# rlav440/pyCamSet

Hardware: AMD Instinct MI355X
Metric: residual+Jacobian rows/sec (higher is better)
Workload: dtype f64; 1 GPU; rig-32 (BASELINE config 3): 32 cams x 200 poses x 486 keys, 998401 detections, chain template; detections_total=998401, detections_per_gpu=998401, row_len_P=21, collective_in_step=none, parallelism=obs-shard x1

## Files before the change

pycamset_amd/csrc/ba_device.hpp:

```cpp
#pragma once
#ifndef __HIPCC_RTC__
#include <hip/hip_runtime.h>

#include <cstdint>
#else
#include "ba_rtc_prelude.hpp"
#endif

namespace pcs {

constexpr int CHAIN_TEMPLATE = 0;
constexpr int CHAIN_SELF = 1;
constexpr int CHAIN_FREE = 2;

__host__ __device__ constexpr int chain_P(int chain) { return chain == CHAIN_TEMPLATE ? 21 : chain == CHAIN_SELF ? 24 : 18; }

constexpr int CAM_STRIDE = 48;
constexpr int POSE_STRIDE = 40;
constexpr int CAM_R = 9, CAM_T = 18, CAM_DR = 21;
constexpr int POSE_R = 0, POSE_T = 9, POSE_DR = 12;

struct DetTable {
    const uint32_t *packed;
    const int32_t *cam, *img, *key;
// ... 260 lines not shown
                for (int aa = 0; aa < 3; ++aa) J[i * P + 15 + aa] = S[i][0] * Qr[0 * 3 + aa] + S[i][1] * Qr[1 * 3 + aa] + S[i][2] * Qr[2 * 3 + aa];
#pragma unroll
                for (int c = 0; c < 3; ++c) J[i * P + 18 + c] = S[i][c];
            }
            if constexpr (CHAIN == CHAIN_SELF) {
#pragma unroll
                for (int i = 0; i < 2; ++i)
#pragma unroll
                    for (int c = 0; c < 3; ++c)
                        J[i * P + 21 + c] = S[i][0] * ps[POSE_R + 0 * 3 + c] + S[i][1] * ps[POSE_R + 1 * 3 + c] + S[i][2] * ps[POSE_R + 2 * 3 + c];
            }
        }
    }
}

template <int CHAIN, typename SlabPtrC, typename SlabPtrP, typename MatPtr, typename VecPtr>
__device__ __forceinline__ void eval_detection_jvp(SlabPtrC cs, SlabPtrP ps, const double X0, const double X1, const double X2, MatPtr M, VecPtr vi,
                                                   VecPtr vet, VecPtr vpt, const double vX0, const double vX1, const double vX2, double &du, double &dv) {
    double Xw0, Xw1, Xw2, dW0, dW1, dW2;
    if constexpr (CHAIN != CHAIN_FREE) {
        const double r0 = ps[POSE_R + 0], r1 = ps[POSE_R + 1], r2 = ps[POSE_R + 2];
        const double r3 = ps[POSE_R + 3], r4 = ps[POSE_R + 4], r5 = ps[POSE_R + 5];
        const double r6 = ps[POSE_R + 6], r7 = ps[POSE_R + 7], r8 = ps[POSE_R + 8];
        Xw0 = r0 * X0 + r1 * X1 + r2 * X2 + ps[POSE_T + 0];
        Xw1 = r3 * X0 + r4 * X1 + r5 * X2 + ps[POSE_T + 1];
        Xw2 = r6 * X0 + r7 * X1 + r8 * X2 + ps[POSE_T + 2];
        dW0 = M[9] * X0 + M[10] * X1 + M[11] * X2 + vpt[0];
        dW1 = M[12] * X0 + M[13] * X1 + M[14] * X2 + vpt[1];
        dW2 = M[15] * X0 + M[16] * X1 + M[17] * X2 + vpt[2];
        if constexpr (CHAIN == CHAIN_SELF) {
// ... 38 lines not shown
```

pycamset_amd/csrc/ba_normal.hpp:

```cpp
#pragma once
#include <hip/hip_runtime.h>

#include <cstddef>

#include "ba_device.hpp"
#include "ba_matfree.hpp"

namespace pcs {

struct NormalArgs {
    DetTable tab;
    const int32_t *order;
    const void *cam_slab, *pose_slab, *points;
    double *H;
    double *HB, *HC;
    double *g;
    double *cost;
    int32_t ldA, ldB, tb;
    int32_t trail_group;
    int64_t trail_off;
    int64_t n, n_tiles;
    int64_t extr_off, pose_off, point_off;
    int64_t n_params;
    int32_t tiles_per_wave;
    const int32_t *stop;
    const int32_t *sel;
    int64_t alt;
    double *part;
    const int32_t *seg_base;
    int32_t loss;
    double inv_f_scale, f_scale_sq;
    double *wave_cost;
    int32_t debug;
    const double *inv_sigma;
};

constexpr int PASS_SHARED = 0, PASS_CAMKEY = 1, PASS_IMGKEY = 2;
constexpr int NORMAL_R = 30;
constexpr int normal_shared_cols(int chain) { return chain == CHAIN_FREE ? 15 : 21; }
constexpr int normal_slots(int chain, int pass) {
    return pass == PASS_SHARED ? normal_shared_cols(chain) + 1 : pass == PASS_CAMKEY ? 19 : 9;
}
constexpr int normal_mfmas(int chain, int pass) { return (pass == PASS_SHARED && chain != CHAIN_FREE) ? 2 : 1; }
constexpr int normal_slot_stride(int rows) { return 2 * rows * 8 + 8; }
constexpr int normal_lds_bytes(int chain, int pass, int rows) { return normal_slots(chain, pass) * normal_slot_stride(rows) + 128; }

template <int CHAIN, int PASS>
__host__ __device__ __forceinline__ constexpr int slot_col(int s) {
    constexpr int NS = normal_shared_cols(CHAIN);
    if (PASS == PASS_SHARED) return s < NS ? s : NORMAL_R;
    if (PASS == PASS_CAMKEY) return s < 15 ? s : s < 18 ? NS + (s - 15) : NORMAL_R;
    return s < 6 ? 15 + s : NS + (s - 6);
}

template <int CHAIN, int PASS>
__host__ __device__ __forceinline__ int window_slot(int w, int j) {
    if (PASS == PASS_SHARED) {
        if (CHAIN == CHAIN_FREE) return j;
        if (w == 1) return j;
        const int g = w == 0 ? 0 : 8;
        return j < 8 ? g + j : j < 14 ? 16 + (j - 8) : -1;
    }
    if (PASS == PASS_CAMKEY) {
        if (w == 0) return j < 3 ? 15 + j : j == 3 ? 18 : j - 4;
        return j < 3 ? 15 + j : j < 6 ? 12 + (j - 3) : -1;
    }
    if (w == 0) return j < 6 ? j : -1;
    return j < 3 ? 6 + j : -1;
}
template <int CHAIN, int PASS> constexpr int n_windows() { return (PASS == PASS_SHARED) ? (CHAIN == CHAIN_FREE ? 1 : 3) : 2; }
template <int CHAIN, int PASS> __host__ __device__ __forceinline__ constexpr int mfma_a(int m) { return PASS == PASS_SHARED ? (CHAIN == CHAIN_FREE ? 0 : m == 0 ? 0 : 2) : 0; }
template <int CHAIN, int PASS> __host__ __device__ __forceinline__ constexpr int mfma_b(int m) { return PASS == PASS_SHARED ? (CHAIN == CHAIN_FREE ? 0 : m == 0 ? 1 : 2) : 1; }

template <int CHAIN, int PASS>
__host__ __device__ __forceinline__ bool entry_kept(int m, int i, int j, int &sa, int &sb) {
    sa = window_slot<CHAIN, PASS>(mfma_a<CHAIN, PASS>(m), i);
    sb = window_slot<CHAIN, PASS>(mfma_b<CHAIN, PASS>(m), j);
    if (sa < 0 || sb < 0) return false;
    if (PASS == PASS_SHARED) {
        if (CHAIN == CHAIN_FREE) return i <= j;
        if (m == 0) return i >= 8 || i <= j;
        return i <= j && !(i < 8 && j >= 8);
    }
    if (PASS == PASS_CAMKEY) {
        if (i < 3) return j >= 3 || i <= j;
        return j < 3;
    }
    return true;
}

template <int CHAIN, int PASS>
__host__ __device__ __forceinline__ int entry_descriptor(const int m, const int lane, const int r, const int tg) {
    constexpr bool HAS_POSE = CHAIN != CHAIN_FREE;
    constexpr int NS = normal_shared_cols(CHAIN);
    auto col_group = [](const int lc) -> int { return lc == NORMAL_R ? 4 : lc < 9 ? 0 : lc < 15 ? 1 : (HAS_POSE && lc < NS) ? 2 : 3; };
    auto col_offset = [](const int lc) -> int { return lc == NORMAL_R ? 0 : lc < 9 ? lc : lc < 15 ? lc - 9 : (HAS_POSE && lc < NS) ? lc - 15 : lc - NS; };
    int sa, sb;
    const bool keep = entry_kept<CHAIN, PASS>(m, (lane >> 4) + 4 * r, lane & 15, sa, sb);
    const int la = slot_col<CHAIN, PASS>(keep ? sa : 0), lb = slot_col<CHAIN, PASS>(keep ? sb : 0);
    int gR = col_group(la), oR = col_offset(la), gC = col_group(lb), oC = col_offset(lb);
    const bool pose = PASS == PASS_SHARED && (gR == 2 || gC == 2);
    if (gR > gC || (gR == gC && oR > oC)) { int t = gR; gR = gC; gC = t; t = oR; oR = oC; oC = t; }
    int eRow, eCol, eLd, ePtr;
    if (gR == 4) { oR = 0; oC = 0; eRow = 9; eCol = 9; eLd = 15; ePtr = 4; }
    else if (gC == 4) { oC = oR; oR = 0; eRow = 9; eCol = 24 + gR; eLd = 15; ePtr = 3; }
    else if (gR == tg) { eRow = 8; eCol = 9; eLd = 14; ePtr = 2; }
    else if (gC == tg) { eRow = 4 + gR; eCol = 16 + gC; eLd = 13; ePtr = 1; }
    else { eRow = gR; eCol = 16 + gC; eLd = 12; ePtr = 0; }
    return oR | (oC << 4) | (eRow << 8) | (eCol << 13) | (eLd << 18) | (ePtr << 23) | (keep ? 1 << 27 : 0) | (pose ? 1 << 28 : 0);
}

template <int CHAIN, int PASS, int KS>
__device__ __attribute__((noinline)) double2v robust_scale_row(const int kind, const double r0, const double r1, const double inv_f_scale,
                                                               const double f_scale_sq, const double *inv_sigma_tab, const int idx, unsigned char *dst) {
    const double inv_sigma = inv_sigma_tab ? inv_sigma_tab[idx] : 1.0;
    double q0, q1, f0, f1;
    const double s0 = robust_rho<true>(kind, r0 * inv_sigma, inv_f_scale, f_scale_sq, q0, f0) * inv_sigma;
    const double s1 = robust_rho<true>(kind, r1 * inv_sigma, inv_f_scale, f_scale_sq, q1, f1) * inv_sigma;
#pragma unroll
    for (int s = 0; s < normal_slots(CHAIN, PASS); ++s) {
        double *q = reinterpret_cast<double *>(dst + s * KS);
        if (slot_col<CHAIN, PASS>(s) == NORMAL_R) {
            q[0] = f0;
            q[1] = f1;
        } else {
            q[0] *= s0;
            q[1] *= s1;
        }
    }
    return double2v{q0, q1};
}

using d4v = __attribute__((ext_vector_type(4))) double;

template <int CHAIN, int PASS, int ROWS>
__global__ __launch_bounds__(64, 2) void ba_normal_mfma_kernel(const NormalArgs a) {
    static_assert(ROWS == 64 || ROWS == 32, "image holds a whole or half a tile");
    static_assert(PASS == PASS_SHARED || CHAIN != CHAIN_TEMPLATE, "the template chain has no point columns");
    static_assert(PASS != PASS_IMGKEY || CHAIN == CHAIN_SELF, "only the self chain couples poses and points");
    using T = double;
    constexpr int P = chain_P(CHAIN);
    constexpr int P2 = 2 * P;
    constexpr int NSLOT = normal_slots(CHAIN, PASS);
    constexpr int NW = n_windows<CHAIN, PASS>();
    constexpr int NM = normal_mfmas(CHAIN, PASS);
    constexpr int KS = normal_slot_stride(ROWS);
    constexpr int STEPS = ROWS / 2;
    constexpr bool HAS_POSE = CHAIN != CHAIN_FREE;
    using D2 = __attribute__((ext_vector_type(2))) double;

    extern __shared__ __attribute__((aligned(16))) unsigned char lds_image[];
    if (a.stop && *a.stop) return;
    const int lane = threadIdx.x;
    const T *cam_slab = static_cast<const T *>(a.cam_slab);
    const T *pose_slab = static_cast<const T *>(a.pose_slab);
    const T *points = static_cast<const T *>(a.points);

    int rd_off[NW];
#pragma unroll
    for (int w = 0; w < NW; ++w) {
        const int s = window_slot<CHAIN, PASS>(w, lane & 15);
        rd_off[w] = (s < 0 ? 0 : s) * KS + (lane >> 4) * 8;
    }
    const int tg = a.trail_group;
    int ent[NM][4];
#pragma unroll
    for (int m = 0; m < NM; ++m)
#pragma unroll
        for (int r = 0; r < 4; ++r) ent[m][r] = entry_descriptor<CHAIN, PASS>(m, lane, r, tg);
    const bool robust = a.loss != LOSS_LINEAR;
    if (PASS == PASS_SHARED && robust) {
#pragma unroll
        for (int m = 0; m < NM; ++m)
#pragma unroll
            for (int r = 0; r < 4; ++r)
                if (((ent[m][r] >> 23) & 7) == 4) ent[m][r] &= ~(1 << 27);
    }
    double rho_acc = 0.0;
    const int64_t out_shift = (a.sel && *a.sel) ? 8 * a.alt : 0;
    const uint64_t out_ptr = (lane == 1 ? (uint64_t)a.HB : lane == 2 ? (uint64_t)a.HC : lane == 3 ? (uint64_t)a.g : lane == 4 ? (uint64_t)a.cost : (uint64_t)a.H) + (uint64_t)out_shift;
    const int ptr_lo = (int)(uint32_t)out_ptr, ptr_hi = (int)(uint32_t)(out_ptr >> 32);
    int base_tab = lane == 12 ? a.ldA : lane == 13 ? a.ldB : lane == 14 ? a.tb : 0;
    d4v acc[NM];
#pragma unroll
    for (int m = 0; m < NM; ++m) acc[m] = d4v{0.0, 0.0, 0.0, 0.0};

    int run_a = -1, run_b = -1;

    int64_t seg = a.part ? a.seg_base[blockIdx.x] : 0;
    auto flush = [&](const bool everything) {
        if (run_a < 0) return;
        if (a.part) {
            double *slot = a.part + seg * (NM * 256) + lane;
#pragma unroll
            for (int m = 0; m < NM; ++m)
#pragma unroll
                for (int r = 0; r < 4; ++r) {
                    slot[(m * 4 + r) * 64] = acc[m][r];
                    acc[m][r] = 0.0;
                }
            ++seg;
            return;
        }
        if (a.debug & 128) {
#pragma unroll
            for (int m = 0; m < NM; ++m)
#pragma unroll
                for (int r = 0; r < 4; ++r) acc[m][r] = (everything || (ent[m][r] & (1 << 28))) ? 0.0 : acc[m][r];
            return;
        }
        const int cam = PASS == PASS_IMGKEY ? 0 : run_a;
        const int img = PASS == PASS_SHARED ? run_b : run_a;
        const int key = run_b;
        const int base[4] = {9 * cam, (int)a.extr_off + 6 * cam, (int)a.pose_off + 6 * img, (int)a.point_off + 3 * key};
#pragma unroll
        for (int g = 0; g < 4; ++g) {
            const uint32_t b = (uint32_t)__builtin_amdgcn_readfirstlane(base[g]);
            const int rowA = (int)((uint32_t)a.ldA * b), rowB = (int)((uint32_t)a.ldB * b);
            const int col = (int)(b - (g == tg ? (uint32_t)a.trail_off : 0u)), gi = (int)b;
            asm("v_writelane_b32 %0, %1, %2" : "+v"(base_tab) : "s"(rowA), "n"(g));
            asm("v_writelane_b32 %0, %1, %2" : "+v"(base_tab) : "s"(rowB), "n"(4 + g));
            asm("v_writelane_b32 %0, %1, %2" : "+v"(base_tab) : "s"(col), "n"(16 + g));
            asm("v_writelane_b32 %0, %1, %2" : "+v"(base_tab) : "s"(gi), "n"(24 + g));
        }
        {
            const int ent_idx = tg == 2 ? img : key;
            const int rowC = __builtin_amdgcn_readfirstlane((int)((uint32_t)(a.tb * a.tb) * (uint32_t)ent_idx));
            asm("v_writelane_b32 %0, %1, %2" : "+v"(base_tab) : "s"(rowC), "n"(8));
        }
        uint64_t dst[NM][4];
        int dsc[NM][4];
#pragma unroll
        for (int m = 0; m < NM; ++m)
#pragma unroll
            for (int r = 0; r < 4; ++r) {
                int d = ent[m][r];
                asm volatile("" : "+v"(d));
                const uint32_t ld = (uint32_t)__builtin_amdgcn_ds_bpermute((d >> 16) & (31 << 2), base_tab);
                const uint32_t off = (uint32_t)__builtin_amdgcn_ds_bpermute((d >> 6) & (31 << 2), base_tab) +
                                     (uint32_t)__builtin_amdgcn_ds_bpermute((d >> 11) & (31 << 2), base_tab) +
                                     ((uint32_t)(d & 15) * ld + (uint32_t)((d >> 4) & 15));
                const int psel = (d >> 21) & (7 << 2);
                const uint64_t pb = ((uint64_t)(uint32_t)__builtin_amdgcn_ds_bpermute(psel, ptr_hi) << 32) | (uint32_t)__builtin_amdgcn_ds_bpermute(psel, ptr_lo);
                dst[m][r] = pb + ((uint64_t)off << 3);
                dsc[m][r] = d;
            }
#pragma unroll
        for (int m = 0; m < NM; ++m)
#pragma unroll
            for (int r = 0; r < 4; ++r) {
                const int d = dsc[m][r];
                const bool now = everything || (d & (1 << 28));
                const double s = acc[m][r];
                acc[m][r] = now ? 0.0 : s;
                if (now && (d & (1 << 27)) && s != 0.0 && !(a.debug & 2))
                    __builtin_amdgcn_global_atomic_fadd_f64(reinterpret_cast<__attribute__((address_space(1))) double *>(dst[m][r]), s);
            }
    };

    const int64_t tile0 = (int64_t)blockIdx.x * a.tiles_per_wave;
    const int64_t tile1 = min(tile0 + (int64_t)a.tiles_per_wave, a.n_tiles);
    auto det_index = [&](const int64_t tile) -> int64_t {
        const int64_t i = tile * 64 + lane;
        const int64_t is = i < a.n ? i : a.n - 1;
        return a.order ? a.order[is] : is;
    };
    DetWords nxt_w{};
    double2v nxt_m{};
    if (tile0 < tile1) {
// ... 13 lines not shown
            nxt_w = load_words(a.tab, icn);
            nxt_m = load_uv(a.tab, icn);
        }
        asm volatile("" ::: "memory");
        T u, v;
        T J[P2];
        if (a.debug & 16) {
            u = m.x; v = m.y;
#pragma unroll
            for (int j = 0; j < P2; ++j) J[j] = m.x + (double)j;
        } else {
            const T X0 = points[3 * k], X1 = points[3 * k + 1], X2 = points[3 * k + 2];
            const int c0 = __builtin_amdgcn_readfirstlane(c), im0 = __builtin_amdgcn_readfirstlane(im);
            const bool cam_uni = __all(c == c0), img_uni = !HAS_POSE || __all(im == im0);
            const T *csp = cam_slab + c * CAM_STRIDE, *psp = pose_slab + im * POSE_STRIDE;
            if (PASS == PASS_SHARED && cam_uni && img_uni) {
                const LaneSlab lc{cam_slab[c0 * CAM_STRIDE + min(lane, CAM_STRIDE - 1)]};
                const LaneSlab lp{HAS_POSE ? pose_slab[im0 * POSE_STRIDE + min(lane, POSE_STRIDE - 1)] : 0.0};
                eval_detection<CHAIN, T, true>(lc, lp, X0, X1, X2, u, v, J);
            } else if (PASS == PASS_CAMKEY && cam_uni) {
                const LaneSlab lc{cam_slab[c0 * CAM_STRIDE + min(lane, CAM_STRIDE - 1)]};
                eval_detection<CHAIN, T, true>(lc, psp, X0, X1, X2, u, v, J);
            } else if (PASS == PASS_IMGKEY && img_uni) {
                const LaneSlab lp{pose_slab[im0 * POSE_STRIDE + min(lane, POSE_STRIDE - 1)]};
                eval_detection<CHAIN, T, true>(csp, lp, X0, X1, X2, u, v, J);
            } else {
                eval_detection<CHAIN, T, true>(csp, psp, X0, X1, X2, u, v, J);
            }
        }
        const double r0 = u - m.x, r1 = v - m.y;
        asm volatile("" ::"v"(nxt_w.w0), "v"(nxt_w.w1), "v"(nxt_w.w2), "v"(nxt_m.x), "v"(nxt_m.y));

        const int ka = PASS == PASS_IMGKEY ? im : c, kb = PASS == PASS_SHARED ? im : k;
        const int pa = __shfl_up(ka, 1), pb = __shfl_up(kb, 1);
        const bool starts = valid && (lane == 0 ? (ka != run_a || kb != run_b) : (ka != pa || kb != pb));
        const uint64_t bnd = __ballot(starts);

#pragma unroll
        for (int h = 0; h < 64 / ROWS; ++h) {
            if (!(a.debug & 64) && (ROWS == 64 || (lane >> 5) == h)) {
                unsigned char *dst = lds_image + (lane & (ROWS - 1)) * 16;
#pragma unroll
                for (int s = 0; s < NSLOT; ++s) {
                    const int lc = slot_col<CHAIN, PASS>(s);
                    double *q = reinterpret_cast<double *>(dst + s * KS);
                    q[0] = lc == NORMAL_R ? r0 : J[lc];
                    q[1] = lc == NORMAL_R ? r1 : J[P + lc];
                }
                if (!valid) {
#pragma unroll
                    for (int s = 0; s < NSLOT; ++s) {
                        double *q = reinterpret_cast<double *>(dst + s * KS);
                        q[0] = 0.0;
                        q[1] = 0.0;
                    }
                } else if (robust) {
                    int w_off = (int)offsetof(NormalArgs, inv_sigma);
                    asm volatile("" : "+s"(w_off));
                    using KernArg = const __attribute__((address_space(4))) char *;
                    const double *inv_sigma = *reinterpret_cast<const double *const __attribute__((address_space(4))) *>((KernArg)__builtin_amdgcn_kernarg_segment_ptr() + w_off);
                    const int det = (int)tile * 64 + lane;
                    const double2v q = robust_scale_row<CHAIN, PASS, KS>(a.loss, r0, r1, a.inv_f_scale, a.f_scale_sq, inv_sigma, a.order ? a.order[det] : det, dst);
                    if (PASS == PASS_SHARED) {
                        if (a.loss == LOSS_CAUCHY || a.loss == LOSS_ARCTAN)
                            rho_acc += a.f_scale_sq * robust_rho_transcendental(a.loss, q.x) + a.f_scale_sq * robust_rho_transcendental(a.loss, q.y);
                        else
                            rho_acc += q.x + q.y;
                    }
                }
            }
            __builtin_amdgcn_fence(__ATOMIC_RELEASE, "wavefront");
            __builtin_amdgcn_wave_barrier();
            __builtin_amdgcn_fence(__ATOMIC_ACQUIRE, "wavefront");

            const int d_base = h * ROWS;
            const uint64_t bits = (a.debug & 32) ? 0ull : ROWS == 64 ? bnd : (bnd >> d_base) & 0xffffffffull;
            auto operand = [&](const int w, const int s) { return *reinterpret_cast<const double *>(lds_image + rd_off[w] + s * 32); };
            auto run_mfmas = [&](const double (&x)[NW]) {
#pragma unroll
                for (int mm = 0; mm < NM; ++mm)
                    acc[mm] = __builtin_amdgcn_mfma_f64_16x16x4f64(x[mfma_a<CHAIN, PASS>(mm)], x[mfma_b<CHAIN, PASS>(mm)], acc[mm], 0, 0, 0);
            };
            auto new_run = [&](const int d) {
                const int na = __builtin_amdgcn_readlane(ka, d), nb = __builtin_amdgcn_readlane(kb, d);
                flush(PASS != PASS_SHARED || na != run_a);
                run_a = na;
                run_b = nb;
            };
            const uint32_t lds_base = (uint32_t)(uintptr_t)(__attribute__((address_space(3))) unsigned char *)lds_image;
            auto run_steps = [&](const int s0, const int s1) {
                if (s0 >= s1) return;
                double x[3][NW];
                using LdsD = const __attribute__((address_space(3))) double *;
                uint32_t adr[NW];
#pragma unroll
                for (int w = 0; w < NW; ++w) {
                    adr[w] = lds_base + (uint32_t)rd_off[w] + (uint32_t)s0 * 32u;
                    asm volatile("" : "+v"(adr[w]));
                    x[0][w] = *(LdsD)(uintptr_t)adr[w];
                    x[1][w] = *(LdsD)(uintptr_t)(adr[w] + 32u);
// ... 47 lines not shown
                        run_mfmas(xa);
                        new_run(d0 + 1);
                        run_mfmas(xb);
                    } else {
                        run_mfmas(x);
                    }
                    s0 = sb + 1;
                }
            }
            __builtin_amdgcn_fence(__ATOMIC_RELEASE, "wavefront");
            __builtin_amdgcn_wave_barrier();
            __builtin_amdgcn_fence(__ATOMIC_ACQUIRE, "wavefront");
        }
    }
    flush(true);
    if (PASS == PASS_SHARED && robust) {
        const double c = wave_sum(rho_acc);
        if (lane == 0) {
            if (a.part) a.wave_cost[blockIdx.x] = c;
            else if (c != 0.0 && !(a.debug & 2)) unsafeAtomicAdd(a.cost + out_shift / 8, c);
        }
    }
}

constexpr int IK_COLS = 6;
constexpr int IK_SLOT = 64 * 8 + 16;
constexpr int IK_RUNS = IK_COLS * IK_SLOT;
constexpr int IK_GRAM = IK_RUNS + 65 * 16;
constexpr int normal_imgkey_lds_bytes() { return IK_GRAM + 64 * IK_COLS * 8; }

__global__ __launch_bounds__(64, 3) void ba_normal_imgkey_kernel(const NormalArgs a) {
// ... 168 lines not shown
```

pycamset_amd/csrc/pcs_common.inc:

```

static thread_local std::string g_err;

static int fail(int code, const char *fmt, ...) {
    char buf[512];
    va_list ap;
    va_start(ap, fmt);
    vsnprintf(buf, sizeof buf, fmt, ap);
    va_end(ap);
    g_err = buf;
    return code;
}

#define HIPCHK(expr)                                                                              \
    do {                                                                                          \
        hipError_t _e = (expr);                                                                   \
        if (_e != hipSuccess) return fail(PCS_ERR_HIP, "%s failed: %s (%s:%d)", #expr, hipGetErrorString(_e), __FILE__, __LINE__); \
    } while (0)

static int device_cu_count(int device) {
    static std::atomic<int> cached[64];
    if (device < 0 || device >= 64) return 0;
    int v = cached[device].load();
    if (v == 0) {
        if (hipDeviceGetAttribute(&v, hipDeviceAttributeMultiprocessorCount, device) != hipSuccess) v = 0;
        cached[device].store(v);
    }
    return v;
}

extern "C" {
int pcs_version(void) { return 128; }
const char *pcs_last_error(void) { return g_err.c_str(); }

int pcs_device_count(void) {
    int n = 0;
    if (hipGetDeviceCount(&n) != hipSuccess) return 0;
    return n;
}

int pcs_host_alloc(void **out, int64_t bytes) {
    if (!out || bytes <= 0) return fail(PCS_ERR_ARG, "pcs_host_alloc: bad arguments");
    *out = nullptr;
    HIPCHK(hipHostMalloc(out, (size_t)bytes, hipHostMallocDefault));
    return PCS_OK;
}

// ... 50 lines not shown
```

pycamset_amd/csrc/pcs_engine.hip:

```cpp
#include <hip/hip_ext.h>
#include <hip/hip_runtime.h>

#include <atomic>

#include <algorithm>
#include <array>
#include <cmath>
#include <cstdarg>
#include <cstdint>
#include <cstdio>
#include <cstdlib>
#include <cstring>
#include <initializer_list>
#include <string>
#include <vector>

#include "../../include/pcs_hip.h"
#include "ba_device.hpp"
#include "ba_kernels.hpp"
#include "ba_matfree.hpp"
#include "ba_normal.hpp"
#include "ba_reduce.hpp"
#include "ba_schur.hpp"
#include "ba_lm_fused.hpp"
// ... 93 lines not shown
    int normal_imgkey_product = 1;
    bool matfree_lds = true;
    int n_cu = 256;
    int variant = -1;
    int64_t wgs_per_cu = 0;
    int compact_variant = 1;
    bool xcd_remap = false;
    double tile_locality = 1.0;
    double tile_segments = 1.0;
    int fuse_prep = -1;
    int64_t fuse_prep_max_n = 250000;
    int64_t tiles_per_wg = 0;
    size_t lds_limit = 160 * 1024;
    int64_t spd_timeout_us = 250000;
    int deterministic = 0;
    int loss = 0;
    double f_scale = 1.0;
    int fused_trial = 1;
    std::vector<int32_t> h_order, h_order_ck;
    struct DetPass {
        int64_t n = -1;
        int64_t tpw = 0;
        int32_t n_seg = 0, n_lr = 0, n_grp = 0, n_ent = 0, n_waves = 0;
        int32_t *d_idx = nullptr;
        int64_t off[9] = {};
        double *d_work = nullptr;
        int64_t work_off[4] = {};
    } det_pass[2];
};

// ... 281 lines not shown
        HIPCHK(hipSetDevice(h->device));
        HIPCHK(wait_done_host(h));
        for (auto &e : h->ev)
            if (e) (void)hipEventDestroy(e);
        h->ev.assign(4 * value, nullptr);
        h->ev_has_prep.assign(value, 0);
        for (auto &e : h->ev) HIPCHK(hipEventCreate(&e));
        h->ev_ring = value;
        h->ev_count = 0;
        h->events_valid = false;
    } else if (!strcmp(key, "fused_trial")) {
        h->fused_trial = value != 0;
    } else if (!strcmp(key, "deterministic")) {
        if (value < 0 || value > 1) return fail(PCS_ERR_ARG, "deterministic must be 0 or 1");
        h->deterministic = (int)value;
    } else if (!strcmp(key, "spd_timeout_us")) {
        if (value < 1 || value > 60000000) return fail(PCS_ERR_ARG, "spd_timeout_us must be in [1, 60000000]");
        h->spd_timeout_us = value;
    } else if (!strcmp(key, "tiles_per_wg")) {
        if (value < 0 || value > (1 << 20)) return fail(PCS_ERR_ARG, "tiles_per_wg out of range");
        h->tiles_per_wg = value;
    } else {
        return fail(PCS_ERR_ARG, "pcs_set_option: unknown key '%s'", key);
    }
    return PCS_OK;
}

static_assert(PCS_LOSS_LINEAR == LOSS_LINEAR && PCS_LOSS_HUBER == LOSS_HUBER && PCS_LOSS_SOFT_L1 == LOSS_SOFT_L1 && PCS_LOSS_CAUCHY == LOSS_CAUCHY &&
              PCS_LOSS_ARCTAN == LOSS_ARCTAN, "loss kinds of the C ABI and of ba_device.hpp");
int pcs_set_loss(pcs_engine *h, int kind, double f_scale) {
// ... 219 lines not shown
    switch (chain) {
        case CHAIN_TEMPLATE: return launch_matfree_c<CHAIN_TEMPLATE, false>(op, a, grid, 0, s);
        case CHAIN_SELF: return launch_matfree_c<CHAIN_SELF, false>(op, a, grid, 0, s);
        default: return launch_matfree_c<CHAIN_FREE, false>(op, a, grid, 0, s);
    }
}

template <int CHAIN, int PASS>
static hipError_t launch_normal_p(int rows, const NormalArgs &a, dim3 grid, hipStream_t s) {
    if (rows == 32) hipLaunchKernelGGL((ba_normal_mfma_kernel<CHAIN, PASS, 32>), grid, dim3(64), normal_lds_bytes(CHAIN, PASS, 32), s, a);
    else hipLaunchKernelGGL((ba_normal_mfma_kernel<CHAIN, PASS, 64>), grid, dim3(64), normal_lds_bytes(CHAIN, PASS, 64), s, a);
    return hipGetLastError();
}

static hipError_t launch_normal(int chain, int pass, int rows, const NormalArgs &a, dim3 grid, hipStream_t s) {
    if (pass == PASS_SHARED) {
        switch (chain) {
            case CHAIN_TEMPLATE: return launch_normal_p<CHAIN_TEMPLATE, PASS_SHARED>(rows, a, grid, s);
            case CHAIN_SELF: return launch_normal_p<CHAIN_SELF, PASS_SHARED>(rows, a, grid, s);
            default: return launch_normal_p<CHAIN_FREE, PASS_SHARED>(rows, a, grid, s);
        }
    }
    if (pass == PASS_CAMKEY)
        return chain == CHAIN_SELF ? launch_normal_p<CHAIN_SELF, PASS_CAMKEY>(rows, a, grid, s) : launch_normal_p<CHAIN_FREE, PASS_CAMKEY>(rows, a, grid, s);
    return launch_normal_p<CHAIN_SELF, PASS_IMGKEY>(rows, a, grid, s);
}

template <typename E>
__global__ void gather_rows_kernel(const int32_t *__restrict__ order, const E *__restrict__ src, E *__restrict__ dst, int64_t n) {
    const int64_t i = (int64_t)blockIdx.x * blockDim.x + threadIdx.x;
// ... 325 lines not shown
                const pcs_engine::DetPass &D = h->det_pass[pass];
                if ((int64_t)grid.x != D.n_waves) return fail(PCS_ERR_STATE, "deterministic mode: launch geometry and segment table disagree");
                a.part = D.d_work + D.work_off[0];
                a.seg_base = D.d_idx + D.off[0];
                a.wave_cost = D.d_work + D.work_off[3];
                e = launch_normal(h->chain, pass, h->normal_rows, a, grid, s);
                if (e == hipSuccess) {
                    ReduceArgs ra{};
                    ra.part = a.part; ra.Q = D.d_work + D.work_off[1]; ra.G = D.d_work + D.work_off[2];
                    ra.lr_ptr = D.d_idx + D.off[1]; ra.lr_segs = D.d_idx + D.off[2]; ra.lr_ka = D.d_idx + D.off[3]; ra.lr_kb = D.d_idx + D.off[4];
                    ra.grp_ptr = D.d_idx + D.off[5]; ra.cam_ptr = D.d_idx + D.off[6]; ra.ent_ptr = D.d_idx + D.off[7]; ra.ent_runs = D.d_idx + D.off[8];
                    ra.n_lr = D.n_lr; ra.n_grp = D.n_grp; ra.n_cams = (int32_t)h->n_cams; ra.n_ent = D.n_ent; ra.n_waves = D.n_waves;
                    e = launch_reduce(h->chain, pass, a, ra, s);
                }
            } else {
                e = launch_normal(h->chain, pass, h->normal_rows, a, grid, s);
            }
        }
        if (e != hipSuccess) return fail(PCS_ERR_HIP, "normal-equations kernel launch failed: %s", hipGetErrorString(e));
    }
    if (timed) {
        HIPCHK(hipEventRecord(ev[3], s));
        ++h->ev_count;
        h->events_valid = true;
    }
    HIPCHK(mark_done(h, s));
    return PCS_OK;
}

static int enqueue_eval(pcs_engine *h, const double *d_prm, void *d_resid, void *d_out, bool compact, hipStream_t s) {
    if (h->det.n <= 0) return fail(PCS_ERR_STATE, "no detections set");
// ... 594 lines not shown
```

Baseline: 32.26 billion rows/s.

## Accumulate shared-pass normal equations in a 16-column twist basis, fold back per run

Adds a twist-basis shared pass: each detection's Jacobian is formed against 15 columns (intrinsics plus a 6-dof combined-rigid twist), so the MFMA Gram product uses one 16-wide window instead of three windows and two MFMAs. Per run, a noinline fold routine maps the twist Gram back to the camera/pose parameter columns using LDS scratch and per-run rotation data, then issues atomics. It is enabled by default for non-free chains in the non-deterministic path. It trades cheaper per-row Jacobian and MFMA work for extra per-run fold cost, LDS use and atomics. The metric here is residual+Jacobian rows, so it is unclear whether the normal pass is even timed.

```diff
diff --git a/pycamset_amd/csrc/ba_device.hpp b/pycamset_amd/csrc/ba_device.hpp
--- a/pycamset_amd/csrc/ba_device.hpp
+++ b/pycamset_amd/csrc/ba_device.hpp
@@ -298,6 +298,65 @@
     }
 }
 
+constexpr int NORMAL_TWIST_COLS = 16;
+template <int CHAIN, typename SlabPtrC, typename SlabPtrP>
+__device__ __forceinline__ void eval_detection_twist(SlabPtrC cs, SlabPtrP ps, const double X0, const double X1, const double X2, double &u, double &v,
+                                                     double (&J)[2 * NORMAL_TWIST_COLS]) {
+    static_assert(CHAIN != CHAIN_FREE, "the free chain has one rigid transform: nothing to share");
+    using T = double;
+    constexpr int P = NORMAL_TWIST_COLS;
+    const T r0 = ps[POSE_R + 0], r1 = ps[POSE_R + 1], r2 = ps[POSE_R + 2];
+    const T r3 = ps[POSE_R + 3], r4 = ps[POSE_R + 4], r5 = ps[POSE_R + 5];
+    const T r6 = ps[POSE_R + 6], r7 = ps[POSE_R + 7], r8 = ps[POSE_R + 8];
+    const T Y0 = r0 * X0 + r1 * X1 + r2 * X2, Y1 = r3 * X0 + r4 * X1 + r5 * X2, Y2 = r6 * X0 + r7 * X1 + r8 * X2;
+    const T Xw0 = r0 * X0 + r1 * X1 + r2 * X2 + ps[POSE_T + 0];
+    const T Xw1 = r3 * X0 + r4 * X1 + r5 * X2 + ps[POSE_T + 1];
+    const T Xw2 = r6 * X0 + r7 * X1 + r8 * X2 + ps[POSE_T + 2];
+    const T e0 = cs[CAM_R + 0], e1 = cs[CAM_R + 1], e2 = cs[CAM_R + 2];
+    const T e3 = cs[CAM_R + 3], e4 = cs[CAM_R + 4], e5 = cs[CAM_R + 5];
+    const T e6 = cs[CAM_R + 6], e7 = cs[CAM_R + 7], e8 = cs[CAM_R + 8];
+    const T x = e0 * Xw0 + e1 * Xw1 + e2 * Xw2 + cs[CAM_T + 0];
+    const T y = e3 * Xw0 + e4 * Xw1 + e5 * Xw2 + cs[CAM_T + 1];
+    const T z = e6 * Xw0 + e7 * Xw1 + e8 * Xw2 + cs[CAM_T + 2];
+    const T d0 = e0 * Y0 + e1 * Y1 + e2 * Y2, d1 = e3 * Y0 + e4 * Y1 + e5 * Y2, d2 = e6 * Y0 + e7 * Y1 + e8 * Y2;
+
+    const T fx = cs[0], px = cs[1], fy = cs[2], py = cs[3];
+    const T k0 = cs[4], k1 = cs[5], p0 = cs[6], p1 = cs[7], k2 = cs[8];
+    const T iz = T(1) / z;
+    const T a = x * iz, b = y * iz;
+    const T a2 = a * a, b2 = b * b, ab = a * b;
+    const T r2_ = a2 + b2;
+    const T r4_ = r2_ * r2_;
+    const T r6_ = r4_ * r2_;
+    const T kup = T(1) + k0 * r2_ + k1 * r4_ + k2 * r6_;
+    const T xD = a * kup + T(2) * p0 * ab + p1 * (r2_ + T(2) * a2);
+    const T yD = b * kup + p0 * (r2_ + T(2) * b2) + T(2) * p1 * ab;
+    u = xD * fx + px;
+    v = yD * fy + py;
+    const T dk = k0 + T(2) * k1 * r2_ + T(3) * k2 * r4_;
+    const T ua = fx * (kup + T(2) * a2 * dk + T(2) * p0 * b + T(6) * p1 * a);
+    const T cross = T(2) * (ab * dk + p0 * a + p1 * b);
+    const T ub = fx * cross;
+    const T va = fy * cross;
+    const T vb = fy * (kup + T(2) * b2 * dk + T(6) * p0 * b + T(2) * p1 * a);
+    T Ax[2][3];
+    Ax[0][0] = ua * iz; Ax[0][1] = ub * iz; Ax[0][2] = -(a * ua + b * ub) * iz;
+    Ax[1][0] = va * iz; Ax[1][1] = vb * iz; Ax[1][2] = -(a * va + b * vb) * iz;
+    J[0] = xD;            J[1] = T(1); J[2] = T(0);          J[3] = T(0);
+    J[4] = fx * a * r2_;   J[5] = fx * a * r4_;  J[6] = T(2) * fx * ab;  J[7] = fx * (r2_ + T(2) * a2);  J[8] = fx * a * r6_;
+    J[P + 0] = T(0);      J[P + 1] = T(0);     J[P + 2] = yD;          J[P + 3] = T(1);
+    J[P + 4] = fy * b * r2_; J[P + 5] = fy * b * r4_; J[P + 6] = fy * (r2_ + T(2) * b2); J[P + 7] = T(2) * fy * ab; J[P + 8] = fy * b * r6_;
+#pragma unroll
+    for (int i = 0; i < 2; ++i) {
+        J[i * P + 9] = Ax[i][2] * d1 - Ax[i][1] * d2;
+        J[i * P + 10] = Ax[i][0] * d2 - Ax[i][2] * d0;
+        J[i * P + 11] = Ax[i][1] * d0 - Ax[i][0] * d1;
+#pragma unroll
+        for (int aa = 0; aa < 3; ++aa) J[i * P + 12 + aa] = Ax[i][aa];
+        J[i * P + 15] = T(0);
+    }
+}
+
 template <int CHAIN, typename SlabPtrC, typename SlabPtrP, typename MatPtr, typename VecPtr>
 __device__ __forceinline__ void eval_detection_jvp(SlabPtrC cs, SlabPtrP ps, const double X0, const double X1, const double X2, MatPtr M, VecPtr vi,
                                                    VecPtr vet, VecPtr vpt, const double vX0, const double vX1, const double vX2, double &du, double &dv) {
diff --git a/pycamset_amd/csrc/ba_normal.hpp b/pycamset_amd/csrc/ba_normal.hpp
--- a/pycamset_amd/csrc/ba_normal.hpp
+++ b/pycamset_amd/csrc/ba_normal.hpp
@@ -36,18 +36,23 @@
 };
 
 constexpr int PASS_SHARED = 0, PASS_CAMKEY = 1, PASS_IMGKEY = 2;
+constexpr int PASS_SHARED_TWIST = 3;
+constexpr bool pass_is_shared(int pass) { return pass == PASS_SHARED || pass == PASS_SHARED_TWIST; }
 constexpr int NORMAL_R = 30;
 constexpr int normal_shared_cols(int chain) { return chain == CHAIN_FREE ? 15 : 21; }
 constexpr int normal_slots(int chain, int pass) {
-    return pass == PASS_SHARED ? normal_shared_cols(chain) + 1 : pass == PASS_CAMKEY ? 19 : 9;
+    return pass == PASS_SHARED ? normal_shared_cols(chain) + 1 : pass == PASS_SHARED_TWIST ? NORMAL_TWIST_COLS : pass == PASS_CAMKEY ? 19 : 9;
 }
 constexpr int normal_mfmas(int chain, int pass) { return (pass == PASS_SHARED && chain != CHAIN_FREE) ? 2 : 1; }
 constexpr int normal_slot_stride(int rows) { return 2 * rows * 8 + 8; }
-constexpr int normal_lds_bytes(int chain, int pass, int rows) { return normal_slots(chain, pass) * normal_slot_stride(rows) + 128; }
+constexpr int normal_image_bytes(int chain, int pass, int rows) { return normal_slots(chain, pass) * normal_slot_stride(rows) + 128; }
+constexpr int TWIST_G = 0, TWIST_U = TWIST_G + 16 * 16 * 8, TWIST_W = TWIST_U + 16 * 12 * 8, TWIST_SCRATCH = TWIST_W + 6 * 12 * 8;
+constexpr int normal_lds_bytes(int chain, int pass, int rows) { return normal_image_bytes(chain, pass, rows) + (pass == PASS_SHARED_TWIST ? TWIST_SCRATCH : 0); }
 
 template <int CHAIN, int PASS>
 __host__ __device__ __forceinline__ constexpr int slot_col(int s) {
     constexpr int NS = normal_shared_cols(CHAIN);
+    if (PASS == PASS_SHARED_TWIST) return s < 15 ? s : NORMAL_R;
     if (PASS == PASS_SHARED) return s < NS ? s : NORMAL_R;
     if (PASS == PASS_CAMKEY) return s < 15 ? s : s < 18 ? NS + (s - 15) : NORMAL_R;
     return s < 6 ? 15 + s : NS + (s - 6);
@@ -55,6 +60,7 @@
 
 template <int CHAIN, int PASS>
 __host__ __device__ __forceinline__ int window_slot(int w, int j) {
+    if (PASS == PASS_SHARED_TWIST) return j;
     if (PASS == PASS_SHARED) {
         if (CHAIN == CHAIN_FREE) return j;
         if (w == 1) return j;
@@ -68,15 +74,16 @@
     if (w == 0) return j < 6 ? j : -1;
     return j < 3 ? 6 + j : -1;
 }
-template <int CHAIN, int PASS> constexpr int n_windows() { return (PASS == PASS_SHARED) ? (CHAIN == CHAIN_FREE ? 1 : 3) : 2; }
+template <int CHAIN, int PASS> constexpr int n_windows() { return (PASS == PASS_SHARED_TWIST) ? 1 : (PASS == PASS_SHARED) ? (CHAIN == CHAIN_FREE ? 1 : 3) : 2; }
 template <int CHAIN, int PASS> __host__ __device__ __forceinline__ constexpr int mfma_a(int m) { return PASS == PASS_SHARED ? (CHAIN == CHAIN_FREE ? 0 : m == 0 ? 0 : 2) : 0; }
-template <int CHAIN, int PASS> __host__ __device__ __forceinline__ constexpr int mfma_b(int m) { return PASS == PASS_SHARED ? (CHAIN == CHAIN_FREE ? 0 : m == 0 ? 1 : 2) : 1; }
+template <int CHAIN, int PASS> __host__ __device__ __forceinline__ constexpr int mfma_b(int m) { return PASS == PASS_SHARED_TWIST ? 0 : PASS == PASS_SHARED ? (CHAIN == CHAIN_FREE ? 0 : m == 0 ? 1 : 2) : 1; }
 
 template <int CHAIN, int PASS>
 __host__ __device__ __forceinline__ bool entry_kept(int m, int i, int j, int &sa, int &sb) {
     sa = window_slot<CHAIN, PASS>(mfma_a<CHAIN, PASS>(m), i);
     sb = window_slot<CHAIN, PASS>(mfma_b<CHAIN, PASS>(m), j);
     if (sa < 0 || sb < 0) return false;
+    if (PASS == PASS_SHARED_TWIST) return i <= j;
     if (PASS == PASS_SHARED) {
         if (CHAIN == CHAIN_FREE) return i <= j;
         if (m == 0) return i >= 8 || i <= j;
@@ -89,17 +96,14 @@
     return true;
 }
 
-template <int CHAIN, int PASS>
-__host__ __device__ __forceinline__ int entry_descriptor(const int m, const int lane, const int r, const int tg) {
+template <int CHAIN>
+__host__ __device__ __forceinline__ int column_pair_descriptor(const int la, const int lb, const bool keep, const bool pose_pass, const int tg) {
     constexpr bool HAS_POSE = CHAIN != CHAIN_FREE;
     constexpr int NS = normal_shared_cols(CHAIN);
     auto col_group = [](const int lc) -> int { return lc == NORMAL_R ? 4 : lc < 9 ? 0 : lc < 15 ? 1 : (HAS_POSE && lc < NS) ? 2 : 3; };
     auto col_offset = [](const int lc) -> int { return lc == NORMAL_R ? 0 : lc < 9 ? lc : lc < 15 ? lc - 9 : (HAS_POSE && lc < NS) ? lc - 15 : lc - NS; };
-    int sa, sb;
-    const bool keep = entry_kept<CHAIN, PASS>(m, (lane >> 4) + 4 * r, lane & 15, sa, sb);
-    const int la = slot_col<CHAIN, PASS>(keep ? sa : 0), lb = slot_col<CHAIN, PASS>(keep ? sb : 0);
     int gR = col_group(la), oR = col_offset(la), gC = col_group(lb), oC = col_offset(lb);
-    const bool pose = PASS == PASS_SHARED && (gR == 2 || gC == 2);
+    const bool pose = pose_pass && (gR == 2 || gC == 2);
     if (gR > gC || (gR == gC && oR > oC)) { int t = gR; gR = gC; gC = t; t = oR; oR = oC; oC = t; }
     int eRow, eCol, eLd, ePtr;
     if (gR == 4) { oR = 0; oC = 0; eRow = 9; eCol = 9; eLd = 15; ePtr = 4; }
@@ -109,6 +113,13 @@
     else { eRow = gR; eCol = 16 + gC; eLd = 12; ePtr = 0; }
     return oR | (oC << 4) | (eRow << 8) | (eCol << 13) | (eLd << 18) | (ePtr << 23) | (keep ? 1 << 27 : 0) | (pose ? 1 << 28 : 0);
 }
+template <int CHAIN, int PASS>
+__host__ __device__ __forceinline__ int entry_descriptor(const int m, const int lane, const int r, const int tg) {
+    int sa, sb;
+    const bool keep = entry_kept<CHAIN, PASS>(m, (lane >> 4) + 4 * r, lane & 15, sa, sb);
+    const int la = slot_col<CHAIN, PASS>(keep ? sa : 0), lb = slot_col<CHAIN, PASS>(keep ? sb : 0);
+    return column_pair_descriptor<CHAIN>(la, lb, keep, PASS == PASS_SHARED, tg);
+}
 
 template <int CHAIN, int PASS, int KS>
 __device__ __attribute__((noinline)) double2v robust_scale_row(const int kind, const double r0, const double r1, const double inv_f_scale,
@@ -133,13 +144,118 @@
 
 using d4v = __attribute__((ext_vector_type(4))) double;
 
+__device__ __forceinline__ uint64_t normal_destination(const int d, const int base_tab, const int ptr_lo, const int ptr_hi) {
+    const uint32_t ld = (uint32_t)__builtin_amdgcn_ds_bpermute((d >> 16) & (31 << 2), base_tab);
+    const uint32_t off = (uint32_t)__builtin_amdgcn_ds_bpermute((d >> 6) & (31 << 2), base_tab) +
+                         (uint32_t)__builtin_amdgcn_ds_bpermute((d >> 11) & (31 << 2), base_tab) +
+                         ((uint32_t)(d & 15) * ld + (uint32_t)((d >> 4) & 15));
+    const int psel = (d >> 21) & (7 << 2);
+    const uint64_t pb = ((uint64_t)(uint32_t)__builtin_amdgcn_ds_bpermute(psel, ptr_hi) << 32) | (uint32_t)__builtin_amdgcn_ds_bpermute(psel, ptr_lo);
+    return pb + ((uint64_t)off << 3);
+}
+
+template <int CHAIN>
+__device__ __attribute__((noinline)) d4v twist_fold_run(const d4v g, d4v cam, const double *re_, const double *pp_, const uint32_t scratch,
+                                                        const int base_tab, const int ptr_lo, const int ptr_hi, const int tg, const int debug) {
+    static_assert(CAM_DR - CAM_R == 12 && POSE_DR - POSE_R == 12, "one offset from R to dR in both slabs");
+    using Lds = __attribute__((address_space(3))) double *;
+    using Glob = const __attribute__((address_space(1))) double *;
+    const Glob re = (Glob)(uintptr_t)re_, pp = (Glob)(uintptr_t)pp_;
+    const Lds tw_G = (Lds)(uintptr_t)(scratch + TWIST_G), tw_U = (Lds)(uintptr_t)(scratch + TWIST_U), tw_W = (Lds)(uintptr_t)(scratch + TWIST_W);
+    const int lane = threadIdx.x;
+    {
+        const int sub = lane < 9 ? lane : lane < 18 ? lane - 9 : 0;
+        const int wa = sub / 3, wc = sub - 3 * wa;
+        const Glob rb = (lane >= 9 && lane < 18) ? pp + POSE_R : re;
+        const int sr = wc == 0 ? 2 : wc - 1, sc = wc == 2 ? 0 : wc + 1;
+        const Glob dr = rb + 12 + wa * 9 + sr * 3, rr = rb + sc * 3;
+        const double lm = dr[0] * rr[0] + dr[1] * rr[1] + dr[2] * rr[2];
+        const int a4 = min(lane / 3, 3), row = lane - 3 * (lane / 3);
+        double vk[3];
+#pragma unroll
+        for (int k = 0; k < 3; ++k) {
+            const double mk = __shfl(lm, 9 + min(a4, 2) * 3 + k), tk = pp[POSE_T + k];
+            vk[k] = a4 < 3 ? mk : tk;
+        }
+        const double rmq = re[row * 3] * vk[0] + re[row * 3 + 1] * vk[1] + re[row * 3 + 2] * vk[2];
+        const int c1 = wc == 2 ? 0 : wc + 1, c2 = wc == 0 ? 2 : wc - 1;
+        const double lxq = __shfl(lm, wa * 3 + c1) * __shfl(rmq, 9 + c2) - __shfl(lm, wa * 3 + c2) * __shfl(rmq, 9 + c1);
+        const double re_l = re[min(lane, 8)];
+        if (lane < 9) {
+            tw_W[wc * 12 + wa] = lm;
+            tw_W[(3 + wc) * 12 + wa] = lxq;
+            tw_W[wc * 12 + 6 + wa] = rmq;
+            tw_W[(3 + wa) * 12 + 9 + wc] = re_l;
+        }
+    }
+#pragma unroll
+    for (int r = 0; r < 4; ++r) tw_G[((lane >> 4) + 4 * r) * 16 + (lane & 15)] = g[r];
+    __builtin_amdgcn_fence(__ATOMIC_RELEASE, "wavefront");
+    __builtin_amdgcn_wave_barrier();
+    __builtin_amdgcn_fence(__ATOMIC_ACQUIRE, "wavefront");
+    {
+        const int k = lane >> 2;
+        double gk[6];
+#pragma unroll
+        for (int mm = 0; mm < 6; ++mm) gk[mm] = tw_G[k * 16 + 9 + mm];
+#pragma unroll
+        for (int t = 0; t < 3; ++t) {
+            const int jj = (lane & 3) + 4 * t;
+            double s = 0.0;
+#pragma unroll
+            for (int mm = 0; mm < 6; ++mm) s += gk[mm] * tw_W[mm * 12 + jj];
+            tw_U[k * 12 + jj] = s;
+        }
+    }
+    __builtin_amdgcn_fence(__ATOMIC_RELEASE, "wavefront");
+    __builtin_amdgcn_wave_barrier();
+    __builtin_amdgcn_fence(__ATOMIC_ACQUIRE, "wavefront");
+    auto zt_row = [&](const int i16, const int wcol, const bool mix, const Lds col, const int cs) {
+        double s = 0.0;
+#pragma unroll
+        for (int k = 0; k < 6; ++k) s += tw_W[k * 12 + wcol] * col[(9 + k) * cs];
+        return mix ? s : col[i16 * cs];
+    };
+    {
+        const int j = lane & 15;
+        const bool ju = j >= 9 && j < 15;
+        const Lds col = ju ? tw_U + (j - 9) : tw_G + j;
+        const int cs = ju ? 12 : 16;
+#pragma unroll
+        for (int r = 0; r < 4; ++r) {
+            const int i = (lane >> 4) + 4 * r;
+            const bool mix = i >= 9 && i < 15;
+            cam[r] += zt_row(i, mix ? i - 9 : 0, mix, col, cs);
+        }
+    }
+#pragma unroll
+    for (int t = 0; t < 3; ++t) {
+        const int e = lane + 64 * t;
+        const bool ok = e < 22 * 6;
+        const int row = ok ? e / 6 : 0, pc = ok ? e - 6 * row : 0;
+        const bool mix = row >= 9 && row < 21;
+        const double s = zt_row(row < 9 ? row : 15, mix ? row - 9 : 0, mix, tw_U + 6 + pc, 12);
+        const bool keep = ok && (row < 15 || row == 21 || row - 15 <= pc);
+        const int d = column_pair_descriptor<CHAIN>(row < 21 ? row : NORMAL_R, 15 + pc, keep, false, tg);
+        const uint64_t to = normal_destination(d, base_tab, ptr_lo, ptr_hi);
+        if (keep && s != 0.0 && !(debug & 2))
+            __builtin_amdgcn_global_atomic_fadd_f64(reinterpret_cast<__attribute__((address_space(1))) double *>(to), s);
+    }
+    __builtin_amdgcn_fence(__ATOMIC_RELEASE, "wavefront");
+    __builtin_amdgcn_wave_barrier();
+    __builtin_amdgcn_fence(__ATOMIC_ACQUIRE, "wavefront");
+    return cam;
+}
+
 template <int CHAIN, int PASS, int ROWS>
 __global__ __launch_bounds__(64, 2) void ba_normal_mfma_kernel(const NormalArgs a) {
     static_assert(ROWS == 64 || ROWS == 32, "image holds a whole or half a tile");
-    static_assert(PASS == PASS_SHARED || CHAIN != CHAIN_TEMPLATE, "the template chain has no point columns");
+    static_assert(pass_is_shared(PASS) || CHAIN != CHAIN_TEMPLATE, "the template chain has no point columns");
     static_assert(PASS != PASS_IMGKEY || CHAIN == CHAIN_SELF, "only the self chain couples poses and points");
+    static_assert(PASS != PASS_SHARED_TWIST || CHAIN != CHAIN_FREE, "the free chain has no pose: its shared pass has 16 columns as it is");
     using T = double;
-    constexpr int P = chain_P(CHAIN);
+    constexpr bool SHARED = pass_is_shared(PASS), TWIST = PASS == PASS_SHARED_TWIST;
+    constexpr int P = TWIST ? NORMAL_TWIST_COLS : chain_P(CHAIN);
     constexpr int P2 = 2 * P;
     constexpr int NSLOT = normal_slots(CHAIN, PASS);
     constexpr int NW = n_windows<CHAIN, PASS>();
@@ -169,7 +285,7 @@
 #pragma unroll
         for (int r = 0; r < 4; ++r) ent[m][r] = entry_descriptor<CHAIN, PASS>(m, lane, r, tg);
     const bool robust = a.loss != LOSS_LINEAR;
-    if (PASS == PASS_SHARED && robust) {
+    if (SHARED && robust) {
 #pragma unroll
         for (int m = 0; m < NM; ++m)
 #pragma unroll
@@ -184,6 +300,14 @@
     d4v acc[NM];
 #pragma unroll
     for (int m = 0; m < NM; ++m) acc[m] = d4v{0.0, 0.0, 0.0, 0.0};
+    d4v cam_acc[NM];
+#pragma unroll
+    for (int m = 0; m < NM; ++m) cam_acc[m] = d4v{0.0, 0.0, 0.0, 0.0};
+    const uint32_t tw_scratch = (uint32_t)(uintptr_t)(__attribute__((address_space(3))) unsigned char *)lds_image + (uint32_t)normal_image_bytes(CHAIN, PASS, ROWS);
+    if constexpr (TWIST) {
+        double *const tw_W = reinterpret_cast<double *>(lds_image + normal_image_bytes(CHAIN, PASS, ROWS) + TWIST_W);
+        for (int e = lane; e < 6 * 12; e += 64) tw_W[e] = (e == 3 * 12 + 3 || e == 4 * 12 + 4 || e == 5 * 12 + 5) ? 1.0 : 0.0;
+    }
 
     int run_a = -1, run_b = -1;
 
@@ -206,11 +330,14 @@
 #pragma unroll
             for (int m = 0; m < NM; ++m)
 #pragma unroll
-                for (int r = 0; r < 4; ++r) acc[m][r] = (everything || (ent[m][r] & (1 << 28))) ? 0.0 : acc[m][r];
+                for (int r = 0; r < 4; ++r) {
+                    acc[m][r] = (TWIST || everything || (ent[m][r] & (1 << 28))) ? 0.0 : acc[m][r];
+                    if constexpr (TWIST) cam_acc[m][r] = everything ? 0.0 : cam_acc[m][r];
+                }
             return;
         }
         const int cam = PASS == PASS_IMGKEY ? 0 : run_a;
-        const int img = PASS == PASS_SHARED ? run_b : run_a;
+        const int img = SHARED ? run_b : run_a;
         const int key = run_b;
         const int base[4] = {9 * cam, (int)a.extr_off + 6 * cam, (int)a.pose_off + 6 * img, (int)a.point_off + 3 * key};
 #pragma unroll
@@ -228,6 +355,12 @@
             const int rowC = __builtin_amdgcn_readfirstlane((int)((uint32_t)(a.tb * a.tb) * (uint32_t)ent_idx));
             asm("v_writelane_b32 %0, %1, %2" : "+v"(base_tab) : "s"(rowC), "n"(8));
         }
+        if constexpr (TWIST) {
+            cam_acc[0] = twist_fold_run<CHAIN>(acc[0], cam_acc[0], cam_slab + (int64_t)run_a * CAM_STRIDE + CAM_R, pose_slab + (int64_t)run_b * POSE_STRIDE,
+                                               tw_scratch, base_tab, ptr_lo, ptr_hi, tg, a.debug);
+            acc[0] = d4v{0.0, 0.0, 0.0, 0.0};
+            if (!everything) return;
+        }
         uint64_t dst[NM][4];
         int dsc[NM][4];
 #pragma unroll
@@ -236,13 +369,7 @@
             for (int r = 0; r < 4; ++r) {
                 int d = ent[m][r];
                 asm volatile("" : "+v"(d));
-                const uint32_t ld = (uint32_t)__builtin_amdgcn_ds_bpermute((d >> 16) & (31 << 2), base_tab);
-                const uint32_t off = (uint32_t)__builtin_amdgcn_ds_bpermute((d >> 6) & (31 << 2), base_tab) +
-                                     (uint32_t)__builtin_amdgcn_ds_bpermute((d >> 11) & (31 << 2), base_tab) +
-                                     ((uint32_t)(d & 15) * ld + (uint32_t)((d >> 4) & 15));
-                const int psel = (d >> 21) & (7 << 2);
-                const uint64_t pb = ((uint64_t)(uint32_t)__builtin_amdgcn_ds_bpermute(psel, ptr_hi) << 32) | (uint32_t)__builtin_amdgcn_ds_bpermute(psel, ptr_lo);
-                dst[m][r] = pb + ((uint64_t)off << 3);
+                dst[m][r] = normal_destination(d, base_tab, ptr_lo, ptr_hi);
                 dsc[m][r] = d;
             }
 #pragma unroll
@@ -251,8 +378,9 @@
             for (int r = 0; r < 4; ++r) {
                 const int d = dsc[m][r];
                 const bool now = everything || (d & (1 << 28));
-                const double s = acc[m][r];
-                acc[m][r] = now ? 0.0 : s;
+                double s;
+                if constexpr (TWIST) { s = cam_acc[m][r]; cam_acc[m][r] = now ? 0.0 : s; }
+                else { s = acc[m][r]; acc[m][r] = now ? 0.0 : s; }
                 if (now && (d & (1 << 27)) && s != 0.0 && !(a.debug & 2))
                     __builtin_amdgcn_global_atomic_fadd_f64(reinterpret_cast<__attribute__((address_space(1))) double *>(dst[m][r]), s);
             }
@@ -296,10 +424,22 @@
             const int c0 = __builtin_amdgcn_readfirstlane(c), im0 = __builtin_amdgcn_readfirstlane(im);
             const bool cam_uni = __all(c == c0), img_uni = !HAS_POSE || __all(im == im0);
             const T *csp = cam_slab + c * CAM_STRIDE, *psp = pose_slab + im * POSE_STRIDE;
-            if (PASS == PASS_SHARED && cam_uni && img_uni) {
-                const LaneSlab lc{cam_slab[c0 * CAM_STRIDE + min(lane, CAM_STRIDE - 1)]};
-                const LaneSlab lp{HAS_POSE ? pose_slab[im0 * POSE_STRIDE + min(lane, POSE_STRIDE - 1)] : 0.0};
-                eval_detection<CHAIN, T, true>(lc, lp, X0, X1, X2, u, v, J);
+            if constexpr (TWIST) {
+                if (cam_uni && img_uni) {
+                    const LaneSlab lc{cam_slab[c0 * CAM_STRIDE + min(lane, CAM_STRIDE - 1)]};
+                    const LaneSlab lp{pose_slab[im0 * POSE_STRIDE + min(lane, POSE_STRIDE - 1)]};
+                    eval_detection_twist<CHAIN>(lc, lp, X0, X1, X2, u, v, J);
+                } else {
+                    eval_detection_twist<CHAIN>(csp, psp, X0, X1, X2, u, v, J);
+                }
+            } else if constexpr (PASS == PASS_SHARED) {
+                if (cam_uni && img_uni) {
+                    const LaneSlab lc{cam_slab[c0 * CAM_STRIDE + min(lane, CAM_STRIDE - 1)]};
+                    const LaneSlab lp{HAS_POSE ? pose_slab[im0 * POSE_STRIDE + min(lane, POSE_STRIDE - 1)] : 0.0};
+                    eval_detection<CHAIN, T, true>(lc, lp, X0, X1, X2, u, v, J);
+                } else {
+                    eval_detection<CHAIN, T, true>(csp, psp, X0, X1, X2, u, v, J);
+                }
             } else if (PASS == PASS_CAMKEY && cam_uni) {
                 const LaneSlab lc{cam_slab[c0 * CAM_STRIDE + min(lane, CAM_STRIDE - 1)]};
                 eval_detection<CHAIN, T, true>(lc, psp, X0, X1, X2, u, v, J);
@@ -313,7 +453,7 @@
         const double r0 = u - m.x, r1 = v - m.y;
         asm volatile("" ::"v"(nxt_w.w0), "v"(nxt_w.w1), "v"(nxt_w.w2), "v"(nxt_m.x), "v"(nxt_m.y));
 
-        const int ka = PASS == PASS_IMGKEY ? im : c, kb = PASS == PASS_SHARED ? im : k;
+        const int ka = PASS == PASS_IMGKEY ? im : c, kb = SHARED ? im : k;
         const int pa = __shfl_up(ka, 1), pb = __shfl_up(kb, 1);
         const bool starts = valid && (lane == 0 ? (ka != run_a || kb != run_b) : (ka != pa || kb != pb));
         const uint64_t bnd = __ballot(starts);
@@ -343,7 +483,7 @@
                     const double *inv_sigma = *reinterpret_cast<const double *const __attribute__((address_space(4))) *>((KernArg)__builtin_amdgcn_kernarg_segment_ptr() + w_off);
                     const int det = (int)tile * 64 + lane;
                     const double2v q = robust_scale_row<CHAIN, PASS, KS>(a.loss, r0, r1, a.inv_f_scale, a.f_scale_sq, inv_sigma, a.order ? a.order[det] : det, dst);
-                    if (PASS == PASS_SHARED) {
+                    if (SHARED) {
                         if (a.loss == LOSS_CAUCHY || a.loss == LOSS_ARCTAN)
                             rho_acc += a.f_scale_sq * robust_rho_transcendental(a.loss, q.x) + a.f_scale_sq * robust_rho_transcendental(a.loss, q.y);
                         else
@@ -365,7 +505,7 @@
             };
             auto new_run = [&](const int d) {
                 const int na = __builtin_amdgcn_readlane(ka, d), nb = __builtin_amdgcn_readlane(kb, d);
-                flush(PASS != PASS_SHARED || na != run_a);
+                flush(!SHARED || na != run_a);
                 run_a = na;
                 run_b = nb;
             };
@@ -443,7 +583,7 @@
         }
     }
     flush(true);
-    if (PASS == PASS_SHARED && robust) {
+    if (SHARED && robust) {
         const double c = wave_sum(rho_acc);
         if (lane == 0) {
             if (a.part) a.wave_cost[blockIdx.x] = c;
diff --git a/pycamset_amd/csrc/pcs_common.inc b/pycamset_amd/csrc/pcs_common.inc
--- a/pycamset_amd/csrc/pcs_common.inc
+++ b/pycamset_amd/csrc/pcs_common.inc
@@ -29,7 +29,7 @@
 }
 
 extern "C" {
-int pcs_version(void) { return 128; }
+int pcs_version(void) { return 129; }
 const char *pcs_last_error(void) { return g_err.c_str(); }
 
 int pcs_device_count(void) {
diff --git a/pycamset_amd/csrc/pcs_engine.hip b/pycamset_amd/csrc/pcs_engine.hip
--- a/pycamset_amd/csrc/pcs_engine.hip
+++ b/pycamset_amd/csrc/pcs_engine.hip
@@ -131,6 +131,7 @@
     size_t lds_limit = 160 * 1024;
     int64_t spd_timeout_us = 250000;
     int deterministic = 0;
+    int normal_basis = 1;
     int loss = 0;
     double f_scale = 1.0;
     int fused_trial = 1;
@@ -442,6 +443,9 @@
     } else if (!strcmp(key, "deterministic")) {
         if (value < 0 || value > 1) return fail(PCS_ERR_ARG, "deterministic must be 0 or 1");
         h->deterministic = (int)value;
+    } else if (!strcmp(key, "normal_basis")) {
+        if (value < 0 || value > 1) return fail(PCS_ERR_ARG, "normal_basis must be 0 (parameter columns) or 1 (twist basis)");
+        h->normal_basis = (int)value;
     } else if (!strcmp(key, "spd_timeout_us")) {
         if (value < 1 || value > 60000000) return fail(PCS_ERR_ARG, "spd_timeout_us must be in [1, 60000000]");
         h->spd_timeout_us = value;
@@ -691,6 +695,8 @@
 }
 
 static hipError_t launch_normal(int chain, int pass, int rows, const NormalArgs &a, dim3 grid, hipStream_t s) {
+    if (pass == PASS_SHARED_TWIST)
+        return chain == CHAIN_SELF ? launch_normal_p<CHAIN_SELF, PASS_SHARED_TWIST>(rows, a, grid, s) : launch_normal_p<CHAIN_TEMPLATE, PASS_SHARED_TWIST>(rows, a, grid, s);
     if (pass == PASS_SHARED) {
         switch (chain) {
             case CHAIN_TEMPLATE: return launch_normal_p<CHAIN_TEMPLATE, PASS_SHARED>(rows, a, grid, s);
@@ -1046,7 +1052,8 @@
                     e = launch_reduce(h->chain, pass, a, ra, s);
                 }
             } else {
-                e = launch_normal(h->chain, pass, h->normal_rows, a, grid, s);
+                const bool twist = pass == PASS_SHARED && h->normal_basis == 1 && h->chain != PCS_CHAIN_FREE;
+                e = launch_normal(h->chain, twist ? PASS_SHARED_TWIST : pass, h->normal_rows, a, grid, s);
             }
         }
         if (e != hipSuccess) return fail(PCS_ERR_HIP, "normal-equations kernel launch failed: %s", hipGetErrorString(e));
```

After: 30.77 billion rows/s. 0.954x the previous value.
